# telosnetwork/plonky2_goldibear

Hardware: AMD Instinct MI355X
Metric: proofs/s (higher is better)
Workload: dtype u64; 1 GPU; prove(): 2^20-row Goldilocks dummy circuit (2^19+1 NoopGates), standard_recursion_config_gl with num_challenges=3, Poseidon-12, witness in page-locked host memory, handed over every step -> proof bytes (198432 B); field=goldilocks, log_n=20, cap_height=4, proofs_in_flight_per_gpu=1, witness=in page-locked host memory, handed over every step

## Files before the change

### plonky2_goldibear_amd/csrc/api.hip

```cpp
#include "../../include/goldibear_gpu.h"

#include <hip/hip_runtime.h>

#include <algorithm>
#include <array>
#include <atomic>
#include <condition_variable>
#include <cstdio>
#include <cstring>
#include <exception>
#include <map>
#include <memory>
#include <mutex>
#include <new>
#include <set>
#include <string>
#include <thread>
#include <tuple>
#include <type_traits>
#include <utility>
#include <vector>

#include "bb_field.hpp"
#include "gl_field.hpp"
#include "kernels.hpp"
#include "poseidon2_bb_host.hpp"
#include "poseidon_gl_host.hpp"

using gbk::BbF;
using gbk::GlF;
using gbk::u32;
using gbk::u64;

namespace {

thread_local std::string g_null_ctx_error;

struct DeviceBuf {
    void* p = nullptr;
    size_t bytes = 0;
};

struct ScopeAcc {
    std::vector<std::pair<hipEvent_t, hipEvent_t>> spans;
};

template <class F>
struct TableCache {
    typedef typename F::T T;
    typedef gbk::NttTables<F> Tables;
    typedef gbk::CosetTables<F> Cosets;
    template <class X>
    struct Owner {
        X t{};
        std::vector<void*> owned;
    };
    const T *tw4096_fwd = nullptr, *tw4096_inv = nullptr;
    const T *tw4096_fwd_m = nullptr, *tw4096_inv_m = nullptr;
    std::vector<void*> owned;
    std::map<u32, Owner<Tables>> tables;
    std::map<std::tuple<u32, u32, T, int>, Owner<Cosets>> cosets;
    void release() {
        for (void* p : owned) hipFree(p);
        for (auto& kv : tables) for (void* p : kv.second.owned) hipFree(p);
        for (auto& kv : cosets) for (void* p : kv.second.owned) hipFree(p);
    }
};

struct Stager;

}

struct gb_ctx {
    int device = 0;
    hipStream_t stream = nullptr;
    hipStream_t copy_stream = nullptr;
    std::string err;
// ... 313 lines not shown
}

inline u32 big_work_level(u32 log_n) { return (log_n - gbk::NTT_NATIVE_LOG - 1) / gbk::NTT_OUTER_MAX_BITS; }
gb_status ensure_big_work(gb_ctx* ctx, u32 log_n, u32 rate_bits, size_t es) {
    for (; log_n > gbk::NTT_NATIVE_LOG; log_n -= gbk::ntt_outer_bits(log_n)) {
        const size_t n = (size_t)1 << log_n, per_col = (n + (n << rate_bits)) * es;
        const size_t cols = std::min<size_t>(8, std::max<size_t>(1, ((size_t)8 << 30) / per_col));
        if (gb_status s = ensure(ctx, ctx->big_work[big_work_level(log_n)], cols * per_col)) return s;
    }
    return GB_OK;
}
template <class F>
gb_status cosets_for(gb_ctx* ctx, u32 log_n, u32 rate_bits, typename F::T shift, bool inverse,
                     const typename TableCache<F>::Cosets** out) {
    typedef typename F::T T;
    TableCache<F>& tc = cache<F>(ctx);
    auto key = std::make_tuple(log_n, rate_bits, shift, inverse ? 1 : 0);
    auto it = tc.cosets.find(key);
    if (it != tc.cosets.end()) {
        if (!inverse)
            if (gb_status sw = ensure_big_work(ctx, log_n, rate_bits, sizeof(T))) return sw;
        *out = &it->second.t;
        return GB_OK;
    }
    size_t n = (size_t)1 << log_n;
    size_t nlo = n < 4096 ? n : 4096, nhi = n > 4096 ? n / 4096 : 1;
    u32 nc = 1u << rate_bits;
    T wN = F::two_adic_generator(log_n + rate_bits);
    std::vector<T> lo(nc * nlo), hi(nc * nhi);
    for (u32 c = 0; c < nc; c++) {
        T s = F::mul(shift, F::pow(wN, bitrev32(c, rate_bits)));
        if (inverse) s = F::inv(s);
        std::vector<T> pl = powers<F>(s, nlo), ph = powers<F>(F::pow(s, 4096), nhi);
        std::memcpy(&lo[c * nlo], pl.data(), nlo * sizeof(T));
        std::memcpy(&hi[c * nhi], ph.data(), nhi * sizeof(T));
    }
    typename TableCache<F>::template Owner<typename TableCache<F>::Cosets> set;
    set.t.rate_bits = rate_bits;
    gb_status s;
    if (const u32 K = gbk::ntt_outer_bits(log_n); K && !inverse) {
        if ((s = cosets_for<F>(ctx, log_n - K, rate_bits, F::pow(shift, (u64)1 << K), false, &set.t.sub))) return s;
        if ((s = ensure_big_work(ctx, log_n, rate_bits, sizeof(T)))) return s;
        DeviceBuf& wb = ctx->big_work[big_work_level(log_n)];
        set.t.work = &wb.p; set.t.work_bytes = &wb.bytes;
    }
    if constexpr (!is_goldilocks<F>)
        if (log_n == 22 && !inverse)
            if ((s = cosets_for<F>(ctx, 20, rate_bits + 2, shift, false, &set.t.fine))) return s;
    if ((s = upload(ctx, lo, &set.t.pow_lo, set.owned))) return s;
    if ((s = upload(ctx, hi, &set.t.pow_hi, set.owned))) return s;
    if constexpr (is_goldilocks<F>) {
        if ((s = upload(ctx, times_r(lo), &set.t.pow_lo_m, set.owned))) return s;
        if ((s = upload(ctx, times_r(hi), &set.t.pow_hi_m, set.owned))) return s;
    }
    auto res = tc.cosets.emplace(key, std::move(set));
    *out = &res.first->second.t;
    return GB_OK;
}

static constexpr uint32_t GB_INPUT_DEVICE_FORM = 0x100;
static constexpr uint32_t GB_PUBLIC_INPUT_FLAGS = GB_INPUT_DEVICE | GB_INPUT_P3_REPR;

struct ColSrc {
    const void* base = nullptr;
    const void* const* ptrs = nullptr;
    ColSrc() {}
    ColSrc(const void* b) : base(b) {}
    static ColSrc columns(const void* const* p) { ColSrc s; s.ptrs = p; return s; }
    const char* col(size_t c, size_t col_bytes) const {
        return ptrs ? static_cast<const char*>(ptrs[c]) : static_cast<const char*>(base) + c * col_bytes;
    }
    explicit operator bool() const { return base || ptrs; }
};

bool is_pinned_host(const void* p) {
    hipPointerAttribute_t a;
    if (hipPointerGetAttributes(&a, p) != hipSuccess) { (void)hipGetLastError(); return false; }
    return a.type == hipMemoryTypeHost;
}
bool all_pinned(const ColSrc& src, size_t ncols, size_t col_bytes) {
    if (!src.ptrs) return is_pinned_host(src.base) && is_pinned_host(static_cast<const char*>(src.base) + ncols * col_bytes - 1);
    for (size_t c = 0; c < ncols; c++)
        if (!src.ptrs[c] || !is_pinned_host(src.ptrs[c])) return false;
    return true;
}

struct Stager {
    static constexpr unsigned SLOTS = 4;
    static constexpr size_t PIECE = (size_t)1 << 20, SLOT_MIN = (size_t)64 << 20;
    struct Piece { const char* src; char* dst; size_t bytes; u32 col; };
    std::vector<std::thread> workers;
    std::mutex m;
    std::condition_variable cv_work, cv_done;
    u64 generation = 0;
    unsigned parked = 0;
    bool stop = false;
    std::vector<Piece> pieces;
    std::atomic<size_t> next{0};
    std::unique_ptr<std::atomic<u32>[]> remaining;
    size_t remaining_cap = 0;
    char* ring = nullptr;
    size_t slot_bytes = 0;
    unsigned slot = 0;
    hipEvent_t slot_done[SLOTS] = {};
    bool slot_used[SLOTS] = {};

// ... 830 lines not shown
```

### plonky2_goldibear_amd/csrc/kernels.hpp

```cpp
#pragma once
#include <hip/hip_runtime.h>
#include <stddef.h>
#include <stdint.h>

#include <type_traits>

#include "field_traits.hpp"
#include "gate_set.hpp"
#include "challenge_slices.hpp"

namespace gbk {


struct GlNttTables {
    u32 log_n;
    const u64* tw4096_fwd;
    const u64* tw4096_inv;
    const u64* tw_lo_fwd;
    const u64* tw_hi_fwd;
    const u64* tw_lo_inv;
    const u64* tw_hi_inv;
    u64 n_inv;
    const u64 *tw4096_fwd_m, *tw4096_inv_m, *tw_lo_fwd_m, *tw_hi_fwd_m, *tw_lo_inv_m, *tw_hi_inv_m;
    u64 n_inv_m;
    const u64* tw16k_inv_m;
    const GlNttTables* sub;
    u32 outer_bits;
    const u64* tw_top_fwd;
};
static constexpr u32 NTT_NATIVE_LOG = 22;
static constexpr u32 NTT_OUTER_MAX_BITS = 4;
inline u32 ntt_outer_bits(u32 log_n) { return log_n <= NTT_NATIVE_LOG ? 0 : (log_n - NTT_NATIVE_LOG < NTT_OUTER_MAX_BITS ? log_n - NTT_NATIVE_LOG : NTT_OUTER_MAX_BITS); }

struct GlCosetTables {
    u32 rate_bits;
    const u64* pow_lo;
    const u64* pow_hi;
    const u64 *pow_lo_m, *pow_hi_m;
    const GlCosetTables* sub;
    void* const* work;
    const size_t* work_bytes;
};

struct BbNttTables {
    u32 log_n;
    const u32 *tw4096_fwd, *tw4096_inv, *tw_lo_fwd, *tw_hi_fwd, *tw_lo_inv, *tw_hi_inv;
    u32 n_inv;
    const u32* tw16k_inv;
    const BbNttTables* wide;
    const BbNttTables* sub;
    u32 outer_bits;
    const u32* tw_top_fwd;
};
struct BbCosetTables {
    u32 rate_bits;
    const u32 *pow_lo, *pow_hi;
    const BbCosetTables* fine;
    const BbCosetTables* sub;
    void* const* work;
    const size_t* work_bytes;
};

template <class F>
using NttTables = std::conditional_t<std::is_same<F, GlF>::value, GlNttTables, BbNttTables>;
template <class F>
using CosetTables = std::conditional_t<std::is_same<F, GlF>::value, GlCosetTables, BbCosetTables>;


static constexpr size_t INTT_GROUP = 16;

template <class F>
void intt_columns(const typename F::T* src, typename F::T* coeffs, typename F::T* scratch, size_t ncols, const NttTables<F>& t,
                  hipStream_t stream);
bool bb_intt_columns_canonical(u32* vals, u32* coeffs, u32* scratch, size_t ncols, size_t mont_cols, const BbNttTables& t, hipStream_t stream);
template <class F>
void lde_columns(const typename F::T* coeffs, typename F::T* lde, size_t ncols, const NttTables<F>& t, const CosetTables<F>& ct,
                 hipStream_t stream);
template <class F>
void gather_row(const typename F::T* cols, size_t col_stride, u32 width, u64 index, typename F::T* dst, hipStream_t stream);
template <class F>
void transpose_to_rows(const typename F::T* cols, size_t col_stride, u32 width, u64 rows, typename F::T* dst, hipStream_t stream);
template <class F>
void bitrev_copy(const typename F::T* src, typename F::T* dst, u32 bits, size_t ncols, hipStream_t stream);
template <class F>
void reduce_words(typename F::T* p, size_t count, hipStream_t stream);


void gl_merkle_leaves(const u64* cols, size_t col_stride, u32 width, u64 num_leaves, u64* out, hipStream_t stream);
void gl_merkle_leaves_segment(const u64* cols, size_t col_stride, u32 c_begin, u32 c_end, u64 num_leaves, u64* state, bool last,
                              u32 next_cols, u64* out, hipStream_t stream);
void gl_merkle_level(const u64* in, u64* out, u64 num_out, hipStream_t stream);
// ... 157 lines not shown
```

### plonky2_goldibear_amd/csrc/kernels_ntt16.hip

```cpp
#include "kernels.hpp"
#include "gl_field.hpp"
#include "ntt_passes.hpp"

namespace gbk {

template <int K>
__device__ __forceinline__ u64 mul_pow2(u64 x) {
    static_assert(K >= 0 && K < 96, "shift range");
    if constexpr (K == 0) return x;
    constexpr int k = K % 32, j = K / 32;
    const u32 x0 = (u32)x, x1 = (u32)(x >> 32);
    const u32 y0 = k ? x0 << k : x0;
    const u32 y1 = k ? (x1 << k) | (x0 >> ((32 - k) & 31)) : x1;
    const u32 y2 = k ? x1 >> ((32 - k) & 31) : 0u;
    if constexpr (j == 0) {
        const u64 lo = (u64)y0 | ((u64)y1 << 32), he = ((u64)y2 << 32) - y2;
        u64 t, t2;
        const bool c = __builtin_uaddll_overflow(lo, he, &t);
        const bool d = __builtin_uaddll_overflow(t, gl::EPS, &t2);
        return (c | d) ? t2 : t;
    } else {
        u32 cu, cw, b0, B1, B2, kk;
        u32 hi, s0;
        if constexpr (j == 1) {
            const u32 u0 = __builtin_addc(y0, y1, 0u, &cu);
            hi = u0 + cu;
            s0 = __builtin_addc(y1, y2, cu, &cw);
        } else {
            hi = y0;
            s0 = __builtin_addc(y0, y1, 0u, &cw);
            cw += y2;
        }
        const u32 d0 = __builtin_subc(0u, s0, 0u, &b0);
        const u32 d1 = __builtin_subc(hi, cw, b0, &B1);
        (void)B2;
        const u32 m = 0u - B1;
        const u32 e0 = __builtin_subc(d0, m, 0u, &kk);
        const u32 e1 = d1 - kk;
        return (u64)e0 | ((u64)e1 << 32);
    }
}

template <bool INV, int M>
__device__ __forceinline__ u64 sub_twiddle(u64 a, u64 b) {
    constexpr int e = (INV ? 36 * M : 156 * M) % 192;
    if constexpr (e == 0) return gl::sub(a, b);
    else if constexpr (e < 96) return mul_pow2<e>(gl::sub(a, b));
    else return mul_pow2<e - 96>(gl::sub(b, a));
}

template <bool INV, int H, int J>
__device__ __forceinline__ void bfly(u64& a, u64& b) {
    u64 s = gl::add(a, b);
    b = sub_twiddle<INV, J*(8 / H)>(a, b);
    a = s;
}

template <bool INV>
__device__ __forceinline__ void dft16(u64 (&x)[16]) {
#define B8(J) bfly<INV, 8, J>(x[J], x[J + 8]);
    B8(0) B8(1) B8(2) B8(3) B8(4) B8(5) B8(6) B8(7)
#undef B8
#define B4(O, J) bfly<INV, 4, J>(x[O + J], x[O + J + 4]);
    B4(0, 0) B4(0, 1) B4(0, 2) B4(0, 3) B4(8, 0) B4(8, 1) B4(8, 2) B4(8, 3)
#undef B4
#define B2(O, J) bfly<INV, 2, J>(x[O + J], x[O + J + 2]);
    B2(0, 0) B2(0, 1) B2(4, 0) B2(4, 1) B2(8, 0) B2(8, 1) B2(12, 0) B2(12, 1)
#undef B2
#define B1(O) bfly<INV, 1, 0>(x[O], x[O + 1]);
    B1(0) B1(2) B1(4) B1(6) B1(8) B1(10) B1(12) B1(14)
#undef B1
}

template <bool INV, int K>
__device__ __forceinline__ void dft_small(u64 (&x)[16]) {
    static_assert(K >= 1 && K <= 3, "radix 2, 4 or 8");
    if constexpr (K == 3) {
        bfly<INV, 4, 0>(x[0], x[4]); bfly<INV, 4, 1>(x[1], x[5]); bfly<INV, 4, 2>(x[2], x[6]); bfly<INV, 4, 3>(x[3], x[7]);
    }
    if constexpr (K >= 2) {
#pragma unroll
        for (int o = 0; o < (1 << K); o += 4) {
            bfly<INV, 2, 0>(x[o], x[o + 2]);
            bfly<INV, 2, 1>(x[o + 1], x[o + 3]);
        }
    }
#pragma unroll
    for (int o = 0; o < (1 << K); o += 2) bfly<INV, 1, 0>(x[o], x[o + 1]);
}

template <bool INV, int M>
__device__ __forceinline__ u64 sub_twiddle64(u64 a, u64 b) {
    constexpr int e = (INV ? 153 * M : 39 * M) % 192;
    if constexpr (e == 0) return gl::sub(a, b);
// ... 16 lines not shown
    dft16<INV>(*reinterpret_cast<u64(*)[16]>(&x[0]));
    dft16<INV>(*reinterpret_cast<u64(*)[16]>(&x[16]));
}

template <>
struct Dft<GlF> {
    template <bool INV>
    static __device__ __forceinline__ void dft16(u64 (&x)[16]) { gbk::dft16<INV>(x); }
    template <bool INV, int K>
    static __device__ __forceinline__ void dft_small(u64 (&x)[16]) { gbk::dft_small<INV, K>(x); }
    template <bool INV, int H, int O>
    static __device__ __forceinline__ void layer64(u64* x) { gbk::layer64<INV, H, O>(x); }
};

__global__ __launch_bounds__(THREADS) void k_gl_lde_pb16(u64* __restrict__ lde, const u64* __restrict__ tw4096) {
    __shared__ u64 sh[16 * 272];
    __shared__ u64 tw2[256];
    u64* p = lde + ((size_t)blockIdx.x << 12);
    const u32 tid = threadIdx.x;
    tw2[tid] = tw4096[((brev4(tid >> 4) * (tid & 15)) & 255) * 16];
    u64 x[16];
#pragma unroll
    for (u32 d = 0; d < 16; d++) x[d] = p[d * 256 + tid];
    u64 tw[16];
#pragma unroll
    for (u32 s = 1; s < 16; s++) tw[s] = tw4096[4096 + s * 256 + tid];
    dft16<false>(x);
#pragma unroll
    for (u32 s = 0; s < 16; s++) sh[s * 272 + tid] = s ? gl::mul_mont(x[s], tw[s]) : x[s];
    __syncthreads();
    const u32 hi4 = tid >> 4, lo4 = tid & 15;
#pragma unroll
    for (u32 d = 0; d < 16; d++) x[d] = sh[hi4 * 272 + d * 16 + lo4];
    dft16<false>(x);
    __syncthreads();
#pragma unroll
    for (u32 s = 0; s < 16; s++)
        sh[hi4 * 272 + lo4 * 17 + s] = s ? gl::mul_mont(x[s], tw2[s * 16 + lo4]) : x[s];
    __syncthreads();
#pragma unroll
    for (u32 d = 0; d < 16; d++) x[d] = sh[hi4 * 272 + d * 17 + lo4];
    dft16<false>(x);
    __syncthreads();
#pragma unroll
    for (u32 s = 0; s < 16; s++) sh[tid * 17 + s] = x[s];
    __syncthreads();
#pragma unroll
    for (u32 it = 0; it < 16; it++) {
        const u32 q = it * 256 + tid;
        p[q] = sh[(q >> 4) * 17 + (q & 15)];
    }
}

__global__ __launch_bounds__(THREADS, 3) void k_gl_lde_pa16x2(const u64* __restrict__ coeffs, u64* __restrict__ lde, u32 L, u32 rate_bits,
                                                           const u64* __restrict__ tw4096, const u64* __restrict__ tw_hi,
                                                           const u64* __restrict__ tw_lo, const u64* __restrict__ pow_lo,
                                                           const u64* __restrict__ pow_hi) {
    __shared__ u64 sh[16 * 272];
    __shared__ u64 tw256[256];
    const size_t col = blockIdx.x >> 8;
    const u32 tg = blockIdx.x & 255;
    const u32 tid = threadIdx.x, hi4 = tid >> 4, j = tid & 15;
    const u32 l = (tg << 4) + j;
    const size_t n = (size_t)1 << L;
    const u64* cin = coeffs + col * n + l;
    tw256[tid] = tw4096[tid * 16];
    u64 orig[16];
#pragma unroll
    for (u32 a1 = 0; a1 < 16; a1++) orig[a1] = cin[(size_t)(a1 * 16 + hi4) << 12];
    __syncthreads();
    const u64 ratio = tw_split16<GlF>(tw_hi, tw_lo, 16 * l);
    const u64 f0 = tw_split16<GlF>(tw_hi, tw_lo, brev4(hi4) * l);
    for (u32 c = 0; c < (1u << rate_bits); c++) {
        const u64* ph = pow_hi + (size_t)c * 256 + hi4;
        u64 x[16];
#pragma unroll
        for (u32 a1 = 0; a1 < 16; a1++) x[a1] = ph[a1 * 16];
        const u64 sl = pow_lo[(size_t)c * 4096 + l];
#pragma unroll
        for (u32 a1 = 0; a1 < 16; a1++) x[a1] = gl::mul_mont<true>(orig[a1], x[a1]);
        dft16<false>(x);
#pragma unroll
        for (u32 s = 0; s < 16; s++) sh[s * 272 + tid] = s ? gl::mul_mont<true>(x[s], tw256[(brev4(s) * hi4) & 255]) : x[s];
        __syncthreads();
#pragma unroll
        for (u32 a0 = 0; a0 < 16; a0++) x[a0] = sh[hi4 * 272 + a0 * 16 + j];
        dft16<false>(x);
        u64* out = lde + (col << (L + rate_bits)) + (size_t)c * n + l;
        u64 f = gl::mul_mont_lazy<true>(sl, f0);
#pragma unroll
        for (u32 k = 0; k < 16; k++) {
            out[(size_t)(hi4 * 16 + brev4(k)) << 12] = gl::mul_mont<true>(x[brev4(k)], f);
            if (k < 15) f = gl::mul_mont_lazy<true>(f, ratio);
        }
        __syncthreads();
    }
}

template <int K>
__global__ __launch_bounds__(128 << K, 2) void k_gl_lde_pa32(const u64* __restrict__ coeffs, u64* __restrict__ lde, u32 rate_bits,
                                                             const u64* __restrict__ tw4096, const u64* __restrict__ tw_hi,
                                                             const u64* __restrict__ tw_lo, const u64* __restrict__ pow_lo,
                                                             const u64* __restrict__ pow_hi) {
    constexpr u32 L = 20 + K, A0 = 8u << K , NT = 128u << K, SLOT = NT + 16, ROWS = 256u << K;
    __shared__ u64 sh[32 * SLOT];
    __shared__ u64 twl[ROWS];
    __shared__ u64 phs[2][ROWS];
    const size_t col = blockIdx.x >> 8;
    const u32 tg = blockIdx.x & 255;
    const u32 tid = threadIdx.x, hi = tid >> 4, j = tid & 15;
    const u32 l = (tg << 4) + j;
    const size_t n = (size_t)1 << L;
    const u64* cin = coeffs + col * n + l;
    for (u32 i = tid; i < ROWS; i += NT) {
        twl[i] = tw4096[i << (4 - K)];
        phs[0][i] = pow_hi[i];
    }
    u64 orig[32];
#pragma unroll
    for (u32 a1 = 0; a1 < 32; a1++) orig[a1] = cin[(size_t)(a1 * A0 + hi) << 12];
    __syncthreads();
    const u64 ratio = tw_split16<GlF>(tw_hi, tw_lo, 32 * l);
    const u32 ncosets = 1u << rate_bits;
    u64 sl_next = pow_lo[l];
    for (u32 c = 0; c < ncosets; c++) {
        const u64 sl = sl_next;
        u64 nph[ROWS / NT];
        if (c + 1 < ncosets) {
#pragma unroll
            for (u32 k = 0; k < ROWS / NT; k++) nph[k] = pow_hi[(size_t)(c + 1) * ROWS + tid + k * NT];
            sl_next = pow_lo[(size_t)(c + 1) * 4096 + l];
        }
        const u64* ph = phs[c & 1] + hi;
        u64 x[32];
#pragma unroll
        for (u32 a1 = 0; a1 < 32; a1++) x[a1] = ph[a1 * A0];
#pragma unroll
        for (u32 a1 = 0; a1 < 32; a1++) x[a1] = gl::mul_mont<true>(orig[a1], x[a1]);
        dft32<false>(x);
#pragma unroll
        for (u32 s = 0; s < 32; s++) sh[s * SLOT + tid] = s ? gl::mul_mont<true>(x[s], twl[(brevk(s, 5) * hi) & (ROWS - 1)]) : x[s];
        __syncthreads();
        u64* out = lde + (col << (L + rate_bits)) + (size_t)c * n + l;
        if constexpr (K == 2) {
#pragma unroll
            for (u32 a0 = 0; a0 < 32; a0++) x[a0] = sh[hi * SLOT + a0 * 16 + j];
            dft32<false>(x);
// ... 94 lines not shown
    for (u32 a = 0; a < R; a++) orig[a] = cin[(size_t)a << 12];
    const u32 ncosets = 1u << rate_bits;
    const u64 ratio = tw_split16<GlF>(tw_hi, tw_lo, l);
    for (u32 c = 0; c < ncosets; c++) {
        const u64* ph = pow_hi + ((size_t)c << K);
        u64 x[16];
#pragma unroll
        for (u32 a = 0; a < R; a++) x[a] = a ? gl::mul_mont(orig[a], ph[a]) : orig[a];
        dft_small<false, K>(x);
        u64* out = lde + (col << (L + rate_bits)) + (size_t)c * n + l;
        u64 f = pow_lo[(size_t)c * 4096 + l];
#pragma unroll
        for (u32 k = 0; k < R; k++) {
            out[(size_t)brevk(k, K) << 12] = gl::mul_mont(x[brevk(k, K)], f);
            if (k + 1 < R) f = gl::mul_mont_lazy(f, ratio);
        }
    }
}

__global__ __launch_bounds__(THREADS) void k_gl_lde_pa16x1(const u64* __restrict__ coeffs, u64* __restrict__ lde, u32 rate_bits,
                                                           const u64* __restrict__ tw_hi, const u64* __restrict__ tw_lo,
                                                           const u64* __restrict__ pow_lo, const u64* __restrict__ pow_hi) {
    constexpr u32 L = 16;
    const size_t col = blockIdx.x >> 4;
    const u32 l = ((blockIdx.x & 15) << 8) + threadIdx.x;
    const size_t n = (size_t)1 << L;
    const u64* cin = coeffs + col * n + l;
    u64 orig[16];
#pragma unroll
    for (u32 a = 0; a < 16; a++) orig[a] = cin[(size_t)a << 12];
    const u32 ncosets = 1u << rate_bits;
    const u64 ratio = tw_split16<GlF>(tw_hi, tw_lo, l);
    for (u32 c = 0; c < ncosets; c++) {
        const u64* ph = pow_hi + (size_t)c * 16;
        u64 x[16];
#pragma unroll
        for (u32 a = 0; a < 16; a++) x[a] = a ? gl::mul_mont(orig[a], ph[a]) : orig[a];
        dft16<false>(x);
        u64* out = lde + (col << (L + rate_bits)) + (size_t)c * n + l;
        u64 f = pow_lo[(size_t)c * 4096 + l];
#pragma unroll
        for (u32 k = 0; k < 16; k++) {
            out[(size_t)brev4(k) << 12] = gl::mul_mont(x[brev4(k)], f);
            if (k < 15) f = gl::mul_mont_lazy(f, ratio);
        }
    }
}


void lde_pa_r16(const u64* coeffs, u64* lde, size_t ncols, const GlNttTables& t, const GlCosetTables& ct, hipStream_t stream) {
    const u32 L = t.log_n;
    if (L == 20) {
        hipLaunchKernelGGL(k_gl_lde_pa16x2, dim3((u32)(ncols << 8)), dim3(THREADS), 0, stream, coeffs, lde, L, ct.rate_bits,
                           t.tw4096_fwd_m, t.tw_hi_fwd_m, t.tw_lo_fwd_m, ct.pow_lo_m, ct.pow_hi_m);
        return;
    }
    if (L == 21 || L == 22) {
        if (L == 21)
            hipLaunchKernelGGL(k_gl_lde_pa32<1>, dim3((u32)(ncols << 8)), dim3(256), 0, stream, coeffs, lde, ct.rate_bits, t.tw4096_fwd_m,
                               t.tw_hi_fwd_m, t.tw_lo_fwd_m, ct.pow_lo_m, ct.pow_hi_m);
        else
            hipLaunchKernelGGL(k_gl_lde_pa32<2>, dim3((u32)(ncols << 8)), dim3(512), 0, stream, coeffs, lde, ct.rate_bits, t.tw4096_fwd_m,
                               t.tw_hi_fwd_m, t.tw_lo_fwd_m, ct.pow_lo_m, ct.pow_hi_m);
        return;
    }
#define GB_PAS(KK)                                                                                                        \
    hipLaunchKernelGGL(k_gl_lde_pa16xs<KK>, dim3((u32)(ncols << (4 + KK))), dim3(THREADS), 0, stream, coeffs, lde, ct.rate_bits, \
                       t.tw4096_fwd_m, t.tw_hi_fwd_m, t.tw_lo_fwd_m, ct.pow_lo_m, ct.pow_hi_m)
    if (L >= 13 && L <= 15) {
        const dim3 grid((u32)(ncols << 4));
        if (L == 13) hipLaunchKernelGGL(k_gl_lde_pa_small<1>, grid, dim3(THREADS), 0, stream, coeffs, lde, ct.rate_bits, t.tw_hi_fwd_m, t.tw_lo_fwd_m, ct.pow_lo_m, ct.pow_hi_m);
        if (L == 14) hipLaunchKernelGGL(k_gl_lde_pa_small<2>, grid, dim3(THREADS), 0, stream, coeffs, lde, ct.rate_bits, t.tw_hi_fwd_m, t.tw_lo_fwd_m, ct.pow_lo_m, ct.pow_hi_m);
        if (L == 15) hipLaunchKernelGGL(k_gl_lde_pa_small<3>, grid, dim3(THREADS), 0, stream, coeffs, lde, ct.rate_bits, t.tw_hi_fwd_m, t.tw_lo_fwd_m, ct.pow_lo_m, ct.pow_hi_m);
        return;
    }
    if (L == 17) { GB_PAS(1); return; }
    if (L == 18) { GB_PAS(2); return; }
    if (L == 19) { GB_PAS(3); return; }
#undef GB_PAS
    if (L == 16)
        hipLaunchKernelGGL(k_gl_lde_pa16x1, dim3((u32)(ncols << 4)), dim3(THREADS), 0, stream, coeffs, lde, ct.rate_bits,
                           t.tw_hi_fwd_m, t.tw_lo_fwd_m, ct.pow_lo_m, ct.pow_hi_m);
}

void lde_pb_r16(u64* lde, size_t ntiles, const GlNttTables& t, hipStream_t stream) {
    hipLaunchKernelGGL(k_gl_lde_pb16, dim3((u32)ntiles), dim3(THREADS), 0, stream, lde, t.tw4096_fwd_m);
}

GB_INSTANTIATE_NTT(GlF)

}
```

### plonky2_goldibear_amd/csrc/gl_field.hpp

```cpp
#pragma once
#include <hip/hip_runtime.h>
#include <stdint.h>

namespace gl {

typedef unsigned long long u64;
typedef unsigned int u32;

static constexpr u64 P = 0xFFFFFFFF00000001ULL;
static constexpr u64 EPS = 0xFFFFFFFFULL;
static constexpr u64 GENERATOR = 7;
static constexpr u64 TWO_ADIC_GEN_32 = 1753635133440165772ULL;

__host__ __device__ __forceinline__ u64 canon(u64 x) { return x >= P ? x - P : x; }

#if defined(__HIPCC__)
__device__ __forceinline__ u64 add(u64 a, u64 b) {
    u32 c0, c1, d0, d1;
    u32 s0 = __builtin_addc((u32)a, (u32)b, 0u, &c0);
    u32 s1 = __builtin_addc((u32)(a >> 32), (u32)(b >> 32), c0, &c1);
    u32 t0 = __builtin_addc(s0, 0xFFFFFFFFu, 0u, &d0);
    u32 t1 = __builtin_addc(s1, 0u, d0, &d1);
    const bool sel = (c1 | d1) != 0;
    return sel ? ((u64)t0 | ((u64)t1 << 32)) : ((u64)s0 | ((u64)s1 << 32));
}
__device__ __forceinline__ u64 sub(u64 a, u64 b) {
    u32 b0, b1, k;
    u32 d0 = __builtin_subc((u32)a, (u32)b, 0u, &b0);
    u32 d1 = __builtin_subc((u32)(a >> 32), (u32)(b >> 32), b0, &b1);
    u32 m = 0u - b1;
    u32 e0 = __builtin_subc(d0, m, 0u, &k);
    u32 e1 = d1 - k;
    return (u64)e0 | ((u64)e1 << 32);
}
__device__ __forceinline__ u64 mulhi(u64 a, u64 b) { return __umul64hi(a, b); }
__device__ __forceinline__ u64 mad_carry(u32 a, u32 b, u64 acc, u64& carry) {
    u64 m;
    asm("v_mad_u64_u32 %0, %1, %2, %3, %4" : "=v"(m), "=s"(carry) : "v"(a), "v"(b), "v"(acc));
    return m;
}
__device__ __forceinline__ u32 addc_carry(u32 x, u64 carry) {
    u32 top;
    u64 unused;
    asm("v_addc_co_u32 %0, %1, 0, %2, %3" : "=v"(top), "=s"(unused) : "v"(x), "s"(carry));
    return top;
}
__device__ __forceinline__ u64 mad_one(u32 x, u64 acc) {
    u64 unused;
    asm("v_mad_u64_u32 %0, %1, %2, 1, %0" : "+v"(acc), "=s"(unused) : "v"(x));
    return acc;
}
__device__ __forceinline__ u32 sub_flag(u32 a, u32 b, u64& borrow) {
    u32 d;
    asm("v_sub_co_u32 %0, %1, %2, %3" : "=v"(d), "=s"(borrow) : "v"(a), "v"(b));
    return d;
}
__device__ __forceinline__ u32 subb_flag(u32 a, u32 b, u64 in, u64& borrow) {
    u32 d;
    asm("v_subb_co_u32 %0, %1, %2, %3, %4" : "=v"(d), "=s"(borrow) : "v"(a), "v"(b), "s"(in));
    return d;
}
__device__ __forceinline__ u32 addc_flag(u32 x, u64 in, u64& carry) {
    u32 d;
    asm("v_addc_co_u32 %0, %1, %2, 0, %3" : "=v"(d), "=s"(carry) : "v"(x), "s"(in));
    return d;
}
__device__ __forceinline__ u32 subb_zero(u32 x, u64 in) {
    u32 d;
    u64 unused;
    asm("v_subbrev_co_u32 %0, %1, 0, %2, %3" : "=v"(d), "=s"(unused) : "v"(x), "s"(in));
    return d;
}
#endif
__host__ inline u64 add(u64 a, u64 b) {
    u64 s, u;
    bool c = __builtin_uaddll_overflow(a, b, &s);
    bool c2 = __builtin_uaddll_overflow(s, EPS, &u);
    return (c | c2) ? u : s;
}
__host__ inline u64 sub(u64 a, u64 b) {
    u64 d;
    bool br = __builtin_usubll_overflow(a, b, &d);
    return d - (br ? EPS : 0);
}
__host__ inline u64 mulhi(u64 a, u64 b) { return (u64)(((unsigned __int128)a * b) >> 64); }
__host__ inline u64 mad_carry(u32 a, u32 b, u64 acc, u64& carry) {
    const unsigned __int128 t = (unsigned __int128)a * b + acc;
    carry = (u64)(t >> 64);
    return (u64)t;
}
__host__ inline u32 addc_carry(u32 x, u64 carry) { return x + (u32)(carry & 1); }
__host__ inline u64 mad_one(u32 x, u64 acc) { return acc + x; }
__host__ inline u32 sub_flag(u32 a, u32 b, u64& borrow) { borrow = a < b; return a - b; }
__host__ inline u32 subb_flag(u32 a, u32 b, u64 in, u64& borrow) {
    const u64 d = (u64)a - b - (in & 1);
    borrow = d >> 63;
    return (u32)d;
}
__host__ inline u32 addc_flag(u32 x, u64 in, u64& carry) {
    const u64 d = (u64)x + (in & 1);
    carry = d >> 32;
    return (u32)d;
}
__host__ inline u32 subb_zero(u32 x, u64 in) { return x - (u32)(in & 1); }
__host__ __device__ __forceinline__ u64 neg(u64 a) { return a ? P - a : 0; }

__host__ __device__ __forceinline__ u64 reduce128(u64 lo, u64 hi) {
    u64 hi_hi = hi >> 32, hi_lo = hi & EPS;
    u64 t0 = lo - hi_hi;
    if (lo < hi_hi) t0 -= EPS;
    u64 t1 = (hi_lo << 32) - hi_lo;
    u64 t2 = t0 + t1;
    if (t2 < t0) t2 += EPS;
    return canon(t2);
}
__host__ __device__ __forceinline__ u64 fold128(u32 r0, u32 r1, u32 hl, u32 hh) {
    u32 cs, c1, bw, B, k1, k2;
    u32 s0 = __builtin_addc(hl, hh, 0u, &cs);
    u32 a1 = __builtin_addc(r1, hl, 0u, &c1);
    u32 d0 = __builtin_subc(r0, s0, 0u, &bw);
    u32 d1 = __builtin_subc(a1, cs, bw, &B);
    u32 mC = 0u - c1, mB = 0u - B;
    u32 cl = __builtin_subc(mC, mB, 0u, &k1);
    u32 ch = 0u - k1;
    u32 f0 = __builtin_addc(d0, cl, 0u, &k2);
    u32 f1 = d1 + ch + k2;
    return (u64)f0 | ((u64)f1 << 32);
}
__device__ __forceinline__ u64 fold160(u32 r0, u32 r1, u32 hl, u32 hh, u32 r4) {
    u32 cs, c1, bw, B, k1, k2;
    u32 s0 = __builtin_addc(hl, hh, 0u, &cs);
    u32 s1 = cs + r4;
    u32 a1 = __builtin_addc(r1, hl, 0u, &c1);
    u32 d0 = __builtin_subc(r0, s0, 0u, &bw);
    u32 d1 = __builtin_subc(a1, s1, bw, &B);
    u32 mC = 0u - c1, mB = 0u - B;
    u32 cl = __builtin_subc(mC, mB, 0u, &k1);
    u32 ch = 0u - k1;
    u32 f0 = __builtin_addc(d0, cl, 0u, &k2);
    u32 f1 = d1 + ch + k2;
    return (u64)f0 | ((u64)f1 << 32);
}
template <bool FIVE = false>
__host__ __device__ __forceinline__ void mul_limbs(u64 a, u64 b, u32& r0, u32& r1, u32& hl, u32& hh) {
    u32 a0 = (u32)a, a1 = (u32)(a >> 32), b0 = (u32)b, b1 = (u32)(b >> 32);
    u64 p00 = (u64)a0 * b0;
    u64 p01 = (u64)a0 * b1 + (p00 >> 32);
    if constexpr (!FIVE) {
        u64 carry;
        const u64 m2 = mad_carry(a1, b0, p01, carry);
        const u64 p11 = (u64)a1 * b1 + (m2 >> 32);
        r0 = (u32)p00; r1 = (u32)m2; hl = (u32)p11; hh = addc_carry((u32)(p11 >> 32), carry);
    } else {
        const u64 p10 = (u64)a1 * b0 + (u32)p01;
        const u64 p11 = mad_one((u32)(p10 >> 32), (u64)a1 * b1 + (p01 >> 32));
        r0 = (u32)p00; r1 = (u32)p10; hl = (u32)p11; hh = (u32)(p11 >> 32);
    }
}
// ... 94 lines not shown
```

Measured before the change: 10.96 proofs/s.

## Replace per-coset input scaling in log_n=20 LDE kernel with power-of-two twists

The 2^20 coset LDE kernel no longer multiplies all 16 inputs by pow_hi per coset. Inputs are rescaled once per class of four cosets using a small step table. Within a class, the coset-specific factor is applied as a shift-based power-of-two twist, and the pow_hi factor is folded into the shared stage-twiddle table. This trades 16 Montgomery multiplies per coset for cheap shifts plus a shared-memory table rebuild per coset, at the cost of more intricate algebra and a switch on twist index.

```diff
diff --git a/plonky2_goldibear_amd/csrc/api.hip b/plonky2_goldibear_amd/csrc/api.hip
--- a/plonky2_goldibear_amd/csrc/api.hip
+++ b/plonky2_goldibear_amd/csrc/api.hip
@@ -23,6 +23,7 @@
 
 #include "bb_field.hpp"
 #include "gl_field.hpp"
+#include "gl_lde_scale.hpp"
 #include "kernels.hpp"
 #include "poseidon2_bb_host.hpp"
 #include "poseidon_gl_host.hpp"
@@ -442,6 +443,8 @@
     if constexpr (is_goldilocks<F>) {
         if ((s = upload(ctx, times_r(lo), &set.t.pow_lo_m, set.owned))) return s;
         if ((s = upload(ctx, times_r(hi), &set.t.pow_hi_m, set.owned))) return s;
+        if (log_n == 20 && !inverse)
+            if ((s = upload(ctx, gbk::pa_scale::step_table(shift, log_n, rate_bits), &set.t.pa_step_m, set.owned))) return s;
     }
     auto res = tc.cosets.emplace(key, std::move(set));
     *out = &res.first->second.t;
diff --git a/plonky2_goldibear_amd/csrc/gl_lde_scale.hpp b/plonky2_goldibear_amd/csrc/gl_lde_scale.hpp
--- /dev/null
+++ b/plonky2_goldibear_amd/csrc/gl_lde_scale.hpp
@@ -0,0 +1,99 @@
+#pragma once
+#include <vector>
+
+#include "gl_field.hpp"
+
+namespace gbk {
+
+typedef unsigned long long u64;
+typedef unsigned int u32;
+
+template <int K, bool NEG = false>
+__host__ __device__ __forceinline__ u64 mul_pow2(u64 x) {
+    static_assert(K >= 0 && K < 96, "shift range");
+    if constexpr (K == 0 && !NEG) return x;
+    constexpr int k = K % 32, j = K / 32;
+    const u32 x0 = (u32)x, x1 = (u32)(x >> 32);
+    const u32 y0 = k ? x0 << k : x0;
+    const u32 y1 = k ? (x1 << k) | (x0 >> ((32 - k) & 31)) : x1;
+    const u32 y2 = k ? x1 >> ((32 - k) & 31) : 0u;
+    if constexpr (j == 0) {
+        const u64 lo = (u64)y0 | ((u64)y1 << 32), he = ((u64)y2 << 32) - y2;
+        u64 t, t2;
+        const bool c = __builtin_uaddll_overflow(lo, he, &t);
+        const bool d = __builtin_uaddll_overflow(t, gl::EPS, &t2);
+        const u64 r = (c | d) ? t2 : t;
+        if constexpr (NEG) return gl::sub(0, r);
+        else return r;
+    } else {
+        u32 cu, cw, b0, B1, kk;
+        u32 hi, s0;
+        if constexpr (j == 1) {
+            const u32 u0 = __builtin_addc(y0, y1, 0u, &cu);
+            hi = u0 + cu;
+            s0 = __builtin_addc(y1, y2, cu, &cw);
+        } else {
+            hi = y0;
+            s0 = __builtin_addc(y0, y1, 0u, &cw);
+            cw += y2;
+        }
+        u32 d0, d1;
+        if constexpr (NEG) {
+            d0 = s0;
+            d1 = __builtin_subc(cw, hi, 0u, &B1);
+        } else {
+            d0 = __builtin_subc(0u, s0, 0u, &b0);
+            d1 = __builtin_subc(hi, cw, b0, &B1);
+        }
+        const u32 m = 0u - B1;
+        const u32 e0 = __builtin_subc(d0, m, 0u, &kk);
+        const u32 e1 = d1 - kk;
+        return (u64)e0 | ((u64)e1 << 32);
+    }
+}
+
+namespace pa_scale {
+
+__host__ __device__ constexpr u32 brev(u32 x, u32 bits) {
+    u32 r = 0;
+    for (u32 i = 0; i < bits; i++) r |= ((x >> i) & 1u) << (bits - 1 - i);
+    return r;
+}
+__host__ __device__ constexpr u32 classes(u32 rate_bits) { return rate_bits > 2 ? 1u << (rate_bits - 2) : 1u; }
+__host__ __device__ constexpr u32 class_of(u32 c) { return c >> 2; }
+__host__ __device__ constexpr bool opens_class(u32 c) { return (c & 3) == 0; }
+__host__ __device__ constexpr u32 twist_of(u32 c, u32 rate_bits) { return rate_bits >= 2 ? brev(c & 3, 2) : rate_bits == 1 ? 2 * c : 0; }
+__host__ __device__ constexpr int twist_exp(int t, int a1) { return (39 * t * a1) % 192; }
+
+template <int T, int A1 = 0>
+__host__ __device__ __forceinline__ void twist(u64 (&x)[16], const u64 (&v)[16]) {
+    if constexpr (A1 < 16) {
+        constexpr int e = twist_exp(T, A1);
+        if constexpr (e < 96) x[A1] = mul_pow2<e>(v[A1]);
+        else x[A1] = mul_pow2<e - 96, true>(v[A1]);
+        twist<T, A1 + 1>(x, v);
+    }
+}
+
+__host__ __device__ __forceinline__ u64 stage_factor(u64 tw_m, u64 pow_hi_m) { return gl::mul_mont_lazy<true>(tw_m, pow_hi_m); }
+
+inline std::vector<u64> step_table(u64 shift, u32 log_n, u32 rate_bits) {
+    const u32 nq = classes(rate_bits);
+    std::vector<u64> t((size_t)nq * 16);
+    const u64 G = gl::pow(shift, (u64)1 << (log_n - 4));
+    const u64 order = (u64)1 << (4 + rate_bits);
+    const u64 w = gl::two_adic_generator(4 + rate_bits);
+    for (u32 q = 0; q < nq; q++) {
+        u64 base = G;
+        if (q) base = gl::pow(w, (order + brev(q, rate_bits - 2) - brev(q - 1, rate_bits - 2)) % order);
+        u64 x = 1;
+        for (u32 a1 = 0; a1 < 16; a1++) {
+            t[q * 16 + a1] = gl::to_mont_slow(x);
+            x = gl::mul(x, base);
+        }
+    }
+    return t;
+}
+
+}
+}
diff --git a/plonky2_goldibear_amd/csrc/kernels.hpp b/plonky2_goldibear_amd/csrc/kernels.hpp
--- a/plonky2_goldibear_amd/csrc/kernels.hpp
+++ b/plonky2_goldibear_amd/csrc/kernels.hpp
@@ -37,6 +37,7 @@
     const u64* pow_lo;
     const u64* pow_hi;
     const u64 *pow_lo_m, *pow_hi_m;
+    const u64* pa_step_m;
     const GlCosetTables* sub;
     void* const* work;
     const size_t* work_bytes;
diff --git a/plonky2_goldibear_amd/csrc/kernels_ntt16.hip b/plonky2_goldibear_amd/csrc/kernels_ntt16.hip
--- a/plonky2_goldibear_amd/csrc/kernels_ntt16.hip
+++ b/plonky2_goldibear_amd/csrc/kernels_ntt16.hip
@@ -1,45 +1,9 @@
 #include "kernels.hpp"
 #include "gl_field.hpp"
+#include "gl_lde_scale.hpp"
 #include "ntt_passes.hpp"
 
 namespace gbk {
-
-template <int K>
-__device__ __forceinline__ u64 mul_pow2(u64 x) {
-    static_assert(K >= 0 && K < 96, "shift range");
-    if constexpr (K == 0) return x;
-    constexpr int k = K % 32, j = K / 32;
-    const u32 x0 = (u32)x, x1 = (u32)(x >> 32);
-    const u32 y0 = k ? x0 << k : x0;
-    const u32 y1 = k ? (x1 << k) | (x0 >> ((32 - k) & 31)) : x1;
-    const u32 y2 = k ? x1 >> ((32 - k) & 31) : 0u;
-    if constexpr (j == 0) {
-        const u64 lo = (u64)y0 | ((u64)y1 << 32), he = ((u64)y2 << 32) - y2;
-        u64 t, t2;
-        const bool c = __builtin_uaddll_overflow(lo, he, &t);
-        const bool d = __builtin_uaddll_overflow(t, gl::EPS, &t2);
-        return (c | d) ? t2 : t;
-    } else {
-        u32 cu, cw, b0, B1, B2, kk;
-        u32 hi, s0;
-        if constexpr (j == 1) {
-            const u32 u0 = __builtin_addc(y0, y1, 0u, &cu);
-            hi = u0 + cu;
-            s0 = __builtin_addc(y1, y2, cu, &cw);
-        } else {
-            hi = y0;
-            s0 = __builtin_addc(y0, y1, 0u, &cw);
-            cw += y2;
-        }
-        const u32 d0 = __builtin_subc(0u, s0, 0u, &b0);
-        const u32 d1 = __builtin_subc(hi, cw, b0, &B1);
-        (void)B2;
-        const u32 m = 0u - B1;
-        const u32 e0 = __builtin_subc(d0, m, 0u, &kk);
-        const u32 e1 = d1 - kk;
-        return (u64)e0 | ((u64)e1 << 32);
-    }
-}
 
 template <bool INV, int M>
 __device__ __forceinline__ u64 sub_twiddle(u64 a, u64 b) {
@@ -165,34 +129,45 @@
 __global__ __launch_bounds__(THREADS, 3) void k_gl_lde_pa16x2(const u64* __restrict__ coeffs, u64* __restrict__ lde, u32 L, u32 rate_bits,
                                                            const u64* __restrict__ tw4096, const u64* __restrict__ tw_hi,
                                                            const u64* __restrict__ tw_lo, const u64* __restrict__ pow_lo,
-                                                           const u64* __restrict__ pow_hi) {
+                                                           const u64* __restrict__ pow_hi, const u64* __restrict__ pa_step) {
     __shared__ u64 sh[16 * 272];
-    __shared__ u64 tw256[256];
+    __shared__ u64 twc[256];
     const size_t col = blockIdx.x >> 8;
     const u32 tg = blockIdx.x & 255;
     const u32 tid = threadIdx.x, hi4 = tid >> 4, j = tid & 15;
     const u32 l = (tg << 4) + j;
     const size_t n = (size_t)1 << L;
     const u64* cin = coeffs + col * n + l;
-    tw256[tid] = tw4096[tid * 16];
+    const u64 twb = tw4096[((brev4(hi4) * j) & 255) * 16];
+    twc[tid] = pa_scale::stage_factor(twb, pow_hi[j]);
     u64 orig[16];
 #pragma unroll
     for (u32 a1 = 0; a1 < 16; a1++) orig[a1] = cin[(size_t)(a1 * 16 + hi4) << 12];
     __syncthreads();
     const u64 ratio = tw_split16<GlF>(tw_hi, tw_lo, 16 * l);
     const u64 f0 = tw_split16<GlF>(tw_hi, tw_lo, brev4(hi4) * l);
-    for (u32 c = 0; c < (1u << rate_bits); c++) {
-        const u64* ph = pow_hi + (size_t)c * 256 + hi4;
+    const u32 ncosets = 1u << rate_bits;
+    for (u32 c = 0; c < ncosets; c++) {
+        if (pa_scale::opens_class(c)) {
+            const u64* st = pa_step + pa_scale::class_of(c) * 16;
+#pragma unroll
+            for (u32 a1 = 1; a1 < 16; a1++) orig[a1] = gl::mul_mont<true>(orig[a1], st[a1]);
+        }
+        u64 ph_next = 0;
+        if (c + 1 < ncosets) ph_next = pow_hi[(size_t)(c + 1) * 256 + j];
+        const u64 sl = pow_lo[(size_t)c * 4096 + l];
         u64 x[16];
-#pragma unroll
-        for (u32 a1 = 0; a1 < 16; a1++) x[a1] = ph[a1 * 16];
-        const u64 sl = pow_lo[(size_t)c * 4096 + l];
-#pragma unroll
-        for (u32 a1 = 0; a1 < 16; a1++) x[a1] = gl::mul_mont<true>(orig[a1], x[a1]);
+        switch (pa_scale::twist_of(c, rate_bits)) {
+            case 0: pa_scale::twist<0>(x, orig); break;
+            case 1: pa_scale::twist<1>(x, orig); break;
+            case 2: pa_scale::twist<2>(x, orig); break;
+            default: pa_scale::twist<3>(x, orig); break;
+        }
         dft16<false>(x);
 #pragma unroll
-        for (u32 s = 0; s < 16; s++) sh[s * 272 + tid] = s ? gl::mul_mont<true>(x[s], tw256[(brev4(s) * hi4) & 255]) : x[s];
-        __syncthreads();
+        for (u32 s = 0; s < 16; s++) sh[s * 272 + tid] = gl::mul_mont<true>(x[s], twc[s * 16 + hi4]);
+        __syncthreads();
+        if (c + 1 < ncosets) twc[tid] = pa_scale::stage_factor(twb, ph_next);
 #pragma unroll
         for (u32 a0 = 0; a0 < 16; a0++) x[a0] = sh[hi4 * 272 + a0 * 16 + j];
         dft16<false>(x);
@@ -403,7 +378,7 @@
     const u32 L = t.log_n;
     if (L == 20) {
         hipLaunchKernelGGL(k_gl_lde_pa16x2, dim3((u32)(ncols << 8)), dim3(THREADS), 0, stream, coeffs, lde, L, ct.rate_bits,
-                           t.tw4096_fwd_m, t.tw_hi_fwd_m, t.tw_lo_fwd_m, ct.pow_lo_m, ct.pow_hi_m);
+                           t.tw4096_fwd_m, t.tw_hi_fwd_m, t.tw_lo_fwd_m, ct.pow_lo_m, ct.pow_hi_m, ct.pa_step_m);
         return;
     }
     if (L == 21 || L == 22) {
```

Result: no change. 11.05 proofs/s, median of 6 (+0.9%).

## Stage coset powers in shared memory and use flag-based Goldilocks subtraction

Applied to the files above, without the earlier changes.

The LDE kernel now loads each coset's 256 pow_hi values into a double-buffered shared array, prefetched during the previous coset's iteration. Threads then read shared memory instead of issuing strided global loads per coset. Launch bounds rise from 3 to 4 blocks per CU, which adds register pressure that could cause spills. Field subtraction and mul_pow2 are moved into the shared header and rewritten with inline-asm carry/borrow flag chains to shorten the instruction sequence.

```diff
diff --git a/plonky2_goldibear_amd/csrc/gl_field.hpp b/plonky2_goldibear_amd/csrc/gl_field.hpp
--- a/plonky2_goldibear_amd/csrc/gl_field.hpp
+++ b/plonky2_goldibear_amd/csrc/gl_field.hpp
@@ -24,15 +24,6 @@
     const bool sel = (c1 | d1) != 0;
     return sel ? ((u64)t0 | ((u64)t1 << 32)) : ((u64)s0 | ((u64)s1 << 32));
 }
-__device__ __forceinline__ u64 sub(u64 a, u64 b) {
-    u32 b0, b1, k;
-    u32 d0 = __builtin_subc((u32)a, (u32)b, 0u, &b0);
-    u32 d1 = __builtin_subc((u32)(a >> 32), (u32)(b >> 32), b0, &b1);
-    u32 m = 0u - b1;
-    u32 e0 = __builtin_subc(d0, m, 0u, &k);
-    u32 e1 = d1 - k;
-    return (u64)e0 | ((u64)e1 << 32);
-}
 __device__ __forceinline__ u64 mulhi(u64 a, u64 b) { return __umul64hi(a, b); }
 __device__ __forceinline__ u64 mad_carry(u32 a, u32 b, u64 acc, u64& carry) {
     u64 m;
@@ -58,6 +49,11 @@
 __device__ __forceinline__ u32 subb_flag(u32 a, u32 b, u64 in, u64& borrow) {
     u32 d;
     asm("v_subb_co_u32 %0, %1, %2, %3, %4" : "=v"(d), "=s"(borrow) : "v"(a), "v"(b), "s"(in));
+    return d;
+}
+__device__ __forceinline__ u32 neg_flag(u32 b, u64& borrow) {
+    u32 d;
+    asm("v_sub_co_u32 %0, %1, 0, %2" : "=v"(d), "=s"(borrow) : "v"(b));
     return d;
 }
 __device__ __forceinline__ u32 addc_flag(u32 x, u64 in, u64& carry) {
@@ -97,6 +93,7 @@
     borrow = d >> 63;
     return (u32)d;
 }
+__host__ inline u32 neg_flag(u32 b, u64& borrow) { borrow = b != 0; return 0u - b; }
 __host__ inline u32 addc_flag(u32 x, u64 in, u64& carry) {
     const u64 d = (u64)x + (in & 1);
     carry = d >> 32;
@@ -104,6 +101,56 @@
 }
 __host__ inline u32 subb_zero(u32 x, u64 in) { return x - (u32)(in & 1); }
 __host__ __device__ __forceinline__ u64 neg(u64 a) { return a ? P - a : 0; }
+
+__host__ __device__ __forceinline__ u64 minus_eps_on(u32 d0, u32 d1, u64 c) {
+    u64 co;
+    const u32 e0 = addc_flag(d0, c, co);
+    const u32 e1 = subb_zero(d1, c & ~co);
+    return (u64)e0 | ((u64)e1 << 32);
+}
+__host__ __device__ __forceinline__ u64 sub_flags(u64 a, u64 b) {
+    u64 c0, c;
+    const u32 d0 = sub_flag((u32)a, (u32)b, c0);
+    const u32 d1 = subb_flag((u32)(a >> 32), (u32)(b >> 32), c0, c);
+    return minus_eps_on(d0, d1, c);
+}
+#if defined(__HIPCC__)
+__device__ __forceinline__ u64 sub(u64 a, u64 b) { return sub_flags(a, b); }
+#endif
+
+template <int K>
+__host__ __device__ __forceinline__ u64 mul_pow2(u64 x) {
+    static_assert(K >= 0 && K < 96, "shift range");
+    if constexpr (K == 0) return x;
+    constexpr int k = K % 32, j = K / 32;
+    const u32 x0 = (u32)x, x1 = (u32)(x >> 32);
+    const u32 y0 = k ? x0 << k : x0;
+    const u32 y1 = k ? (x1 << k) | (x0 >> ((32 - k) & 31)) : x1;
+    const u32 y2 = k ? x1 >> ((32 - k) & 31) : 0u;
+    if constexpr (j == 0) {
+        const u64 lo = (u64)y0 | ((u64)y1 << 32), he = ((u64)y2 << 32) - y2;
+        u64 t, t2;
+        const bool c = __builtin_uaddll_overflow(lo, he, &t);
+        const bool d = __builtin_uaddll_overflow(t, EPS, &t2);
+        return (c | d) ? t2 : t;
+    } else {
+        u32 cu, cw;
+        u32 hi, s0;
+        if constexpr (j == 1) {
+            const u32 u0 = __builtin_addc(y0, y1, 0u, &cu);
+            hi = u0 + cu;
+            s0 = __builtin_addc(y1, y2, cu, &cw);
+        } else {
+            hi = y0;
+            s0 = __builtin_addc(y0, y1, 0u, &cw);
+            cw += y2;
+        }
+        u64 b0, B1;
+        const u32 d0 = neg_flag(s0, b0);
+        const u32 d1 = subb_flag(hi, cw, b0, B1);
+        return minus_eps_on(d0, d1, B1);
+    }
+}
 
 __host__ __device__ __forceinline__ u64 reduce128(u64 lo, u64 hi) {
     u64 hi_hi = hi >> 32, hi_lo = hi & EPS;
diff --git a/plonky2_goldibear_amd/csrc/kernels_ntt16.hip b/plonky2_goldibear_amd/csrc/kernels_ntt16.hip
--- a/plonky2_goldibear_amd/csrc/kernels_ntt16.hip
+++ b/plonky2_goldibear_amd/csrc/kernels_ntt16.hip
@@ -4,42 +4,7 @@
 
 namespace gbk {
 
-template <int K>
-__device__ __forceinline__ u64 mul_pow2(u64 x) {
-    static_assert(K >= 0 && K < 96, "shift range");
-    if constexpr (K == 0) return x;
-    constexpr int k = K % 32, j = K / 32;
-    const u32 x0 = (u32)x, x1 = (u32)(x >> 32);
-    const u32 y0 = k ? x0 << k : x0;
-    const u32 y1 = k ? (x1 << k) | (x0 >> ((32 - k) & 31)) : x1;
-    const u32 y2 = k ? x1 >> ((32 - k) & 31) : 0u;
-    if constexpr (j == 0) {
-        const u64 lo = (u64)y0 | ((u64)y1 << 32), he = ((u64)y2 << 32) - y2;
-        u64 t, t2;
-        const bool c = __builtin_uaddll_overflow(lo, he, &t);
-        const bool d = __builtin_uaddll_overflow(t, gl::EPS, &t2);
-        return (c | d) ? t2 : t;
-    } else {
-        u32 cu, cw, b0, B1, B2, kk;
-        u32 hi, s0;
-        if constexpr (j == 1) {
-            const u32 u0 = __builtin_addc(y0, y1, 0u, &cu);
-            hi = u0 + cu;
-            s0 = __builtin_addc(y1, y2, cu, &cw);
-        } else {
-            hi = y0;
-            s0 = __builtin_addc(y0, y1, 0u, &cw);
-            cw += y2;
-        }
-        const u32 d0 = __builtin_subc(0u, s0, 0u, &b0);
-        const u32 d1 = __builtin_subc(hi, cw, b0, &B1);
-        (void)B2;
-        const u32 m = 0u - B1;
-        const u32 e0 = __builtin_subc(d0, m, 0u, &kk);
-        const u32 e1 = d1 - kk;
-        return (u64)e0 | ((u64)e1 << 32);
-    }
-}
+using gl::mul_pow2;
 
 template <bool INV, int M>
 __device__ __forceinline__ u64 sub_twiddle(u64 a, u64 b) {
@@ -162,12 +127,13 @@
     }
 }
 
-__global__ __launch_bounds__(THREADS, 3) void k_gl_lde_pa16x2(const u64* __restrict__ coeffs, u64* __restrict__ lde, u32 L, u32 rate_bits,
+__global__ __launch_bounds__(THREADS, 4) void k_gl_lde_pa16x2(const u64* __restrict__ coeffs, u64* __restrict__ lde, u32 L, u32 rate_bits,
                                                            const u64* __restrict__ tw4096, const u64* __restrict__ tw_hi,
                                                            const u64* __restrict__ tw_lo, const u64* __restrict__ pow_lo,
                                                            const u64* __restrict__ pow_hi) {
     __shared__ u64 sh[16 * 272];
     __shared__ u64 tw256[256];
+    __shared__ u64 phs[2][256];
     const size_t col = blockIdx.x >> 8;
     const u32 tg = blockIdx.x & 255;
     const u32 tid = threadIdx.x, hi4 = tid >> 4, j = tid & 15;
@@ -175,18 +141,20 @@
     const size_t n = (size_t)1 << L;
     const u64* cin = coeffs + col * n + l;
     tw256[tid] = tw4096[tid * 16];
+    phs[0][tid] = pow_hi[tid];
     u64 orig[16];
 #pragma unroll
     for (u32 a1 = 0; a1 < 16; a1++) orig[a1] = cin[(size_t)(a1 * 16 + hi4) << 12];
     __syncthreads();
     const u64 ratio = tw_split16<GlF>(tw_hi, tw_lo, 16 * l);
     const u64 f0 = tw_split16<GlF>(tw_hi, tw_lo, brev4(hi4) * l);
-    for (u32 c = 0; c < (1u << rate_bits); c++) {
-        const u64* ph = pow_hi + (size_t)c * 256 + hi4;
+    const u32 ncosets = 1u << rate_bits;
+    for (u32 c = 0; c < ncosets; c++) {
+        const u64 sl = pow_lo[(size_t)c * 4096 + l];
+        const u64* ph = phs[c & 1] + hi4;
         u64 x[16];
 #pragma unroll
         for (u32 a1 = 0; a1 < 16; a1++) x[a1] = ph[a1 * 16];
-        const u64 sl = pow_lo[(size_t)c * 4096 + l];
 #pragma unroll
         for (u32 a1 = 0; a1 < 16; a1++) x[a1] = gl::mul_mont<true>(orig[a1], x[a1]);
         dft16<false>(x);
@@ -203,6 +171,7 @@
             out[(size_t)(hi4 * 16 + brev4(k)) << 12] = gl::mul_mont<true>(x[brev4(k)], f);
             if (k < 15) f = gl::mul_mont_lazy<true>(f, ratio);
         }
+        if (c + 1 < ncosets) phs[(c + 1) & 1][tid] = pow_hi[(size_t)(c + 1) * 256 + tid];
         __syncthreads();
     }
 }
```

Result: no change. 10.81 proofs/s before, 10.77 proofs/s after (-0.3%).
